# smartroboticslab/okvis2

Measured on AMD Instinct MI355X. Metric: front-end stereo-frames/s (detect+describe+match), 752x480 stereo, higher is better.
Workload: dtype u8/int32 (detect, describe, Hamming) + f64 (match gate); 1 GPU; EuRoC-shaped 752x480 stereo, euroc.yaml front-end params (radius 38, thr 150, <=700 kpts, match thr 60); lanes_per_gpu=1, score_kernels_serialised_across_lanes=False, stereo_frames_per_launch=3072, distinct_frames=256, content=corners, feed=device, cameras_per_multiframe=2, parallelism=frames sharded over 1 GPU(s), no collective

## Files before the change

### okvis2_amd/capi.py

```python
from __future__ import annotations

import ctypes as C
import os

import numpy as np

_HERE = os.path.dirname(os.path.abspath(__file__))
LIB_PATH = os.environ.get("OKVFE_LIB") or os.path.join(_HERE, "libokvfe.so")

OK = 0
ERR_INVALID_ARGUMENT, ERR_NO_DEVICE, ERR_OUT_OF_MEMORY, ERR_UNSUPPORTED, ERR_CAPACITY, ERR_DEVICE, \
    ERR_NOT_READY = 1, 2, 3, 4, 5, 6, 7
ABI_VERSION = 8
DIST_NONE, DIST_RADTAN, DIST_EQUIDISTANT, DIST_RADTAN8 = 0, 1, 2, 3
SCORE_HARRIS, SCORE_AGAST_9_16, SCORE_BRISK_SCALESPACE = 0, 1, 2
DESC_BYTES = 48

KEYPOINT_DTYPE = np.dtype([("x", "<f4"), ("y", "<f4"), ("size", "<f4"), ("angle", "<f4"),
                           ("response", "<f4"), ("octave", "<i4"), ("class_id", "<i4")])
STEREO_MATCH_DTYPE = np.dtype([("k1", "<i4"), ("dist", "<i4"), ("initialisable", "<i4"),
                               ("pad", "<i4"), ("hp_W", "<f8", (4,))])
CAND_DTYPE = np.dtype([("i", "<i4"), ("j", "<i4"), ("dist", "<i4")])
MOTION_MATCH_DTYPE = np.dtype([("k1", "<i4"), ("dist", "<i4"), ("initialisable", "<i4"),
                               ("accepted", "<i4"), ("cos_quality", "<f8"), ("hp_W", "<f8", (4,))])
# ... 48 lines not shown


class DeviceOutputs(C.Structure):
    _fields_ = [("max_keypoints", C.c_int32), ("counts", C.c_void_p), ("keypoints", C.c_void_p),
                ("descriptors", C.c_void_p), ("backproj", C.c_void_p),
                ("backproj_valid", C.c_void_p), ("scores", C.c_void_p),
                ("detect_counts", C.c_void_p), ("candidate_counts", C.c_void_p),
                ("score_pitch", C.c_int32), ("score_strips", C.c_int32)]


EXPORTS = [
    "okvfe_create", "okvfe_destroy", "okvfe_last_error", "okvfe_abi_version",
    "okvfe_set_camera_maps", "okvfe_set_camera", "okvfe_build_awareness_maps",
    "okvfe_detect_describe", "okvfe_detect", "okvfe_detect_ahead", "okvfe_detect_describe_batch_device",
    "okvfe_get_device_outputs", "okvfe_score_column", "okvfe_set_heavy_kernel_chaining", "okvfe_set_keep_score_map", "okvfe_set_internal_lanes", "okvfe_lanes_join", "okvfe_set_fp64_reduction", "okvfe_scale_index", "okvfe_download_image_result", "okvfe_harris_score_device", "okvfe_harris_byte_mover_device",
    "okvfe_match_stereo_batch_device", "okvfe_match_stereo", "okvfe_hamming_candidates",
    "okvfe_hamming_argmin", "okvfe_popcnt_xor", "okvfe_gather_block_bytes",
    "okvfe_pack_gather_block_device", "okvfe_match_stereo_blocks_device",
    "okvfe_profile_enable", "okvfe_profile_read", "okvfe_match_motion_stereo_blocks_device",
    "okvfe_detect_batch_device", "okvfe_describe_batch_device", "okvfe_camera_overlap", "okvfe_compute",
    "okvfe_match_motion_stereo", "okvfe_match_to_map",
    "okvfe_format_keypoint_lines", "okvfe_parse_keypoint_lines", "okvfe_fbrisk_mean",
    "okvfe_match_to_map_uninitialised", "okvfe_pack_gather_blocks_device",
    "okvfe_match_stereo_blocks_batch_device", "okvfe_check_capacity",
    "okvfe_detect_describe_batch_host", "okvfe_verify_place_match", "okvfe_fbrisk_transform",
    "okvfe_match_to_map_landmarks", "okvfe_bow_vector", "okvfe_bow_query_l1",
    "okvfe_get_pattern", "okvfe_set_pattern", "okvfe_pattern_kernel_class",
    "okvfe_match_to_map_blocks_device", "okvfe_match_to_map_uninitialised_blocks_device",
    "okvfe_verify_place_blocks_device",
    "okvfe_comm_unique_id", "okvfe_comm_create", "okvfe_comm_wrap", "okvfe_comm_destroy",
    "okvfe_comm_world", "okvfe_comm_rank", "okvfe_comm_last_error", "okvfe_gather_blocks",
    "okvfe_device_alloc", "okvfe_device_free", "okvfe_stream_create", "okvfe_stream_destroy",
    "okvfe_stream_synchronize", "okvfe_copy_to_device", "okvfe_copy_to_host", "okvfe_device_fill",
    "okvfe_set_camera_ext", "okvfe_build_awareness_maps_ext", "okvfe_camera_overlap_ext",
    "okvfe_match_motion_stereo_ext",
    "okvfe_keyframe_coverage_blocks_device", "okvfe_keyframe_coverage", "okvfe_keyframe_decision",
    "okvfe_landmark_table_check_device", "okvfe_match_to_map_table_blocks_device",
    "okvfe_match_to_map_table_uninitialised_blocks_device",
    "okvfe_ransac3d2d_consensus_blocks_device", "okvfe_remove_outliers_blocks_device",
    "okvfe_match_motion_stereo_blocks_batch_device",
    "okvfe_place_landmark_set", "okvfe_place_claims_blocks_device", "okvfe_place_consensus_blocks_device",
    "okvfe_place_hessian_blocks_device",
    "okvfe_vocabulary_check", "okvfe_bow_vectors_blocks_device", "okvfe_place_query_blocks_device",
    "okvfe_bow_database_add_blocks_device", "okvfe_bow_database_check_device",
    "okvfe_stereo_insert_blocks_device",
    "okvfe_ransac2d2d_consensus_blocks_device",
    "okvfe_overlap_pairs_blocks_device", "okvfe_overlap_fraction", "okvfe_motion_frame_order",
    "okvfe_tracking_quality",
    "okvfe_imu_propagation", "okvfe_imu_propagation_blocks_device",
]
TEST_HOOKS = [
    "okvfe_test_set_map_table_workspace_limit", "okvfe_test_ransac_chunk_records", "okvfe_test_ransac_ring_records",
    "okvfe_test_ransac2d2d_chunk_records", "okvfe_test_ransac2d2d_ring_records", "okvfe_test_ransac2d2d_id_slot",
    "okvfe_test_place_hessian_chunk_terms", "okvfe_test_context_sizes",
]

STAGES = ["harris", "nms", "sort", "select", "map", "describe", "compact", "match"]

_LIB = None


class LandmarkTable(C.Structure):
    _fields_ = [("n_landmarks", C.c_int32), ("n_observations", C.c_int32), ("n_poses", C.c_int32),
                ("hp_W", C.c_void_p), ("quality", C.c_void_p), ("obs_begin", C.c_void_p),
                ("obs_pose", C.c_void_p), ("obs_desc", C.c_void_p), ("obs_backproj", C.c_void_p),
                ("poses", C.c_void_p)]


class LandmarkPool(C.Structure):
    _fields_ = [("status", C.c_void_p), ("n_desc", C.c_void_p), ("obs_rows", C.c_void_p),
                ("projection", C.c_void_p), ("e_W", C.c_void_p), ("r_W", C.c_void_p)]


class LandmarkTableDevice(C.Structure):
    _fields_ = LandmarkTable._fields_


class LandmarkPoolDevice(C.Structure):
    _fields_ = LandmarkPool._fields_


class StereoInsertDevice(C.Structure):
    _fields_ = [("action", C.c_void_p), ("lm", C.c_void_p), ("landmark_out", C.c_void_p), ("counts", C.c_void_p)]


STEREO_MAX_PAIRS = 16
STEREO_REINIT, STEREO_CREATE, STEREO_OBS0, STEREO_OBS1 = 1, 2, 4, 8


class RansacResultDevice(C.Structure):
    _fields_ = [("n_correspondences", C.c_void_p), ("best_hypothesis", C.c_void_p), ("n_inliers", C.c_void_p),
                ("accepted", C.c_void_p), ("hyp_inliers", C.c_void_p), ("state", C.c_void_p),
                ("distance", C.c_void_p), ("landmark_out", C.c_void_p)]


class Ransac2d2dResultDevice(C.Structure):
    _fields_ = [(n, C.c_void_p) for n in (
        "n_correspondences", "rot_best", "rot_inliers", "rel_best", "rel_inliers", "branch", "removed",
        "total_inliers", "rotation_only", "success",
        "rot_hyp_inliers", "rel_hyp_inliers", "match1", "state", "distance", "landmark1_out")]


class PlaceSetDevice(C.Structure):
    _fields_ = [("n_landmarks", C.c_int32), ("hp", C.c_void_p)]


class PlaceClaimsDevice(C.Structure):
# ... 1043 lines not shown
            self._h, C.byref(database) if database is not None else None, _s(stream)))

    @staticmethod
    def _test_ransac_chunk_records() -> int:
        f = lib().okvfe_test_ransac_chunk_records
        f.restype = C.c_int32
        return int(f())

    @staticmethod
    def _test_place_hessian_chunk_terms() -> int:
        f = lib().okvfe_test_place_hessian_chunk_terms
        f.restype = C.c_int32
        return int(f())

    @staticmethod
    def _test_ransac2d2d_chunk_records() -> int:
        f = lib().okvfe_test_ransac2d2d_chunk_records
        f.restype = C.c_int32
        return int(f())

    @staticmethod
    def _test_ransac_ring_records() -> int:
        f = lib().okvfe_test_ransac_ring_records
        f.restype = C.c_int32
        return int(f())

    @staticmethod
    def _test_ransac2d2d_ring_records() -> int:
        f = lib().okvfe_test_ransac2d2d_ring_records
        f.restype = C.c_int32
        return int(f())

    @staticmethod
    def _test_ransac2d2d_id_slot(landmark_id) -> int:
        f = lib().okvfe_test_ransac2d2d_id_slot
        f.argtypes = [C.c_int32]
        f.restype = C.c_int32
        return int(f(int(landmark_id)))

    def _test_set_map_table_workspace_limit(self, nbytes):
        f = lib().okvfe_test_set_map_table_workspace_limit
        f.argtypes = [C.c_void_p, C.c_uint64]
        self._check(f(self._h, int(nbytes)))

    def _test_context_sizes(self, stream=None) -> dict:
        f = lib().okvfe_test_context_sizes
        f.argtypes = [C.c_void_p, C.c_void_p, C.POINTER(C.c_uint64)]
        out = (C.c_uint64 * 8)()
        self._check(f(self._h, _s(stream), out))
        keys = ("ring_slot_bytes", "ring_dev", "table_ws_bytes", "table_ws_dev", "perm_bytes", "perm_dev",
                "table_ws_entries", "perm_entries")
        return dict(zip(keys, (int(v) for v in out)))

    def verify_place_blocks_device(self, blocks_ptr, n_frames, map_dev, k_min_ptr, dist_min_ptr, stream=None):
        self._check(lib().okvfe_verify_place_blocks_device(
            self._h, _p(blocks_ptr), int(n_frames), C.byref(map_dev), _p(k_min_ptr), _p(dist_min_ptr),
            _s(stream)))

    def keyframe_coverage_blocks_device(self, blocks_ptr, n_frames, landmark_ids_ptr, coverage_ptr, id_set_ptr=None,
                                        n_id_set=0, kptrad=KPTRAD, stream=None):
        self._check(lib().okvfe_keyframe_coverage_blocks_device(
            self._h, _p(blocks_ptr), int(n_frames), _p(landmark_ids_ptr), _p(id_set_ptr), int(n_id_set),
            C.c_double(kptrad), _p(coverage_ptr), _s(stream)))

    def keyframe_coverage(self, keypoints, landmark_ids, id_set=None, kptrad=KPTRAD):
        kps = np.ascontiguousarray(keypoints, dtype=KEYPOINT_DTYPE)
        ids = np.ascontiguousarray(landmark_ids, dtype=np.uint64)
        if len(ids) != len(kps):
            raise ValueError("landmark_ids: one per keypoint")
        s = None if id_set is None else np.ascontiguousarray(id_set, dtype=np.uint64).reshape(-1)
        if s is not None and len(s) == 0:
            s = np.zeros(1, dtype=np.uint64)
            n_set = 0
        else:
            n_set = 0 if s is None else len(s)
        out = np.zeros(1, dtype=COVERAGE_DTYPE)
        self._check(lib().okvfe_keyframe_coverage(self._h, _p(kps) if len(kps) else None, len(kps),
                                                  _p(ids) if len(ids) else None, _p(s), n_set,
                                                  C.c_double(kptrad), _p(out)))
        return out[0]

    def overlap_pairs_blocks_device(self, blocks_ptr, block_stride_m, block_stride_c, n_multiframes, n_cams,
                                    landmark_ids_ptr, pair_a, pair_b, counts_ptr, coverage_ptr=None, kptrad=KPTRAD,
                                    stream=None):
        a = np.ascontiguousarray(pair_a, dtype=np.int32).reshape(-1)
        b = np.ascontiguousarray(pair_b, dtype=np.int32).reshape(-1)
        if len(a) != len(b):
            raise ValueError("pair_a / pair_b: one multiframe index each per pair")
        n = len(a)
        self._check(lib().okvfe_overlap_pairs_blocks_device(
            self._h, _p(blocks_ptr), int(block_stride_m), int(block_stride_c), int(n_multiframes), int(n_cams),
            _p(landmark_ids_ptr), _p(a) if n else None, _p(b) if n else None, n, C.c_double(kptrad), _p(counts_ptr),
            _p(coverage_ptr), _s(stream)))

    def gather_block_bytes(self) -> int:
        return int(lib().okvfe_gather_block_bytes(self._h))

    def pack_gather_block_device(self, index, block_ptr, stream=None):
        self._check(lib().okvfe_pack_gather_block_device(self._h, int(index), _p(block_ptr),
                                                         _s(stream)))

    def pack_gather_blocks_device(self, first, n, blocks_ptr, stream=None):
        self._check(lib().okvfe_pack_gather_blocks_device(self._h, int(first), int(n),
                                                          _p(blocks_ptr), _s(stream)))

    def match_stereo_blocks_batch_device(self, blocks0_ptr, blocks1_ptr, n_frames, T0, T1, f0, f1,
# ... 43 lines not shown
```

### okvis2_amd/csrc/capi_match.cpp

```cpp
#include "okvfe_ctx.h"

using namespace okvfe;

extern "C" {

okvfe_status okvfe_match_stereo_batch_device(okvfe_ctx* ctx, const okvfe_stereo_pair* pairs,
                                             int32_t n_pairs, okvfe_stereo_match* matches_dev,
                                             void* stream) {
  if (!ctx) return OKVFE_ERR_INVALID_ARGUMENT;
  if (!pairs || !matches_dev || n_pairs < 1)
    return fail(ctx, OKVFE_ERR_INVALID_ARGUMENT, "okvfe_match_stereo_batch_device: bad argument");
  HIP_TRY(ctx, hipSetDevice(ctx->cfg.device));
  std::vector<PairParams> pp(n_pairs);
  for (int i = 0; i < n_pairs; ++i) {
    if (pairs[i].image0 < 0 || pairs[i].image0 >= ctx->B || pairs[i].image1 < 0 || pairs[i].image1 >= ctx->B ||
        !(pairs[i].f0 > 0.0) || !(pairs[i].f1 > 0.0))
      return fail(ctx, OKVFE_ERR_INVALID_ARGUMENT, "pair %d: image index or focal length out of range", i);
    pp[i] = to_pair_params(pairs[i]);
  }
  std::vector<int> lane_first;
  bool piped = ctx->lanes_pipelined && ctx->lanes_open && ctx->n_layers == 1 && ctx->lane_chunk > 0 &&
               ctx->lanes_used > 1 && (int)ctx->lane_ctx.size() >= ctx->lanes_used && ctx->join_stream;
  if (piped) {
    lane_first.assign(ctx->lanes_used + 1, n_pairs);
// ... 427 lines not shown
                    fn, i1, user[i1], p);
      user[i1] = p;
    }
    rt8 = rt8 || dc.distortion == OKVFE_DIST_RADTAN8;
    okvfe_stereo_pair sp{};
    sp.T_WC0 = T_WC0[p]; sp.T_WC1 = T_WC1[p];
    sp.f0 = sp.f1 = 0.5 * (dc.fu + dc.fv);
    recs[p].pair = to_pair_params(sp);
    recs[p].cam = cam; recs[p].idx0 = i0; recs[p].idx1 = i1; recs[p].pad = 0;
    size_t j = 0;
    while (j < slots.size() && slots[j] != cam) ++j;
    if (j == slots.size()) slots.push_back(cam);
    slot_of[p] = (int)j;
  }
  if (claim && ctx->kp_cap > kMotionClaimMaxKeypoints)
    return fail(ctx, OKVFE_ERR_UNSUPPORTED, "%s: claims need max_keypoints <= %d (this context: %d)", fn,
                kMotionClaimMaxKeypoints, ctx->kp_cap);
  HIP_TRY(ctx, hipSetDevice(ctx->cfg.device));
  hipStream_t s = pick_stream(ctx, stream);
  const BlockLayout L = block_layout(ctx->kp_cap);
  okvfe_status st;
  RingSlot cls(ctx, &ctx->cls_ring, s), rec(ctx, &ctx->pair_ring, s);
  if (ctx->n_layers > 1) {
    std::vector<double> tables(slots.size() * kClassTableDoubles);
    for (size_t j = 0; j < slots.size(); ++j) {
      const DeviceCamera& dc = ctx->h_cams[slots[j]];
      const double f = 0.5 * (dc.fu + dc.fv);
      fill_class_table(tables.data() + j * kClassTableDoubles, f, f, true);
    }
    if ((st = cls.upload(tables.data(), tables.size() * sizeof(double))) != OKVFE_OK) return st;
    for (int p = 0; p < n_pairs; ++p) recs[p].pair.cls = cls.as<double>() + (size_t)slot_of[p] * kClassTableDoubles;
  }
  if ((st = rec.upload(recs.data(), recs.size() * sizeof(MotionPairRecord))) != OKVFE_OK) return st;
  launch_match_motion_pairs(rec.as<MotionPairRecord>(), n_pairs, ctx->d_cams, ctx->w, ctx->h, L,
                            static_cast<const uint8_t*>(blocks0_dev), static_cast<const uint8_t*>(blocks1_dev),
                            skip0_dev, matched1_dev, ctx->kp_cap, ctx->cfg.match_threshold, matches_dev, s, rt8);
  if (claim)
    launch_motion_claim(rec.as<MotionPairRecord>(), n_pairs, L,
                        static_cast<const uint8_t*>(blocks0_dev), ctx->kp_cap, matches_dev, claim->claimed,
                        claim->n_claimed, claim->matched1_out, s);
  HIP_TRY(ctx, hipGetLastError());
  ctx->last_stream = s;
  if ((st = rec.release()) != OKVFE_OK) return st;
  return cls.release();
}

okvfe_status okvfe_match_stereo_blocks_device(okvfe_ctx* ctx, const void* block0_dev, const void* block1_dev,
                                              const okvfe_pose* T_WC0, const okvfe_pose* T_WC1, double f0,
                                              double f1, okvfe_stereo_match* matches_dev, void* stream) {
  return okvfe_match_stereo_blocks_batch_device(ctx, block0_dev, block1_dev, 1, T_WC0, T_WC1, f0, f1, matches_dev,
                                                stream);
}

}
```

### okvis2_amd/csrc/k_match.hip

```cpp
#include "camera_dev.h"
#include <algorithm>
#include <cassert>

#include "okvfe_internal.h"
#include "bow_dev.h"

namespace okvfe {
namespace {

__device__ int g_fp64_tree = 1;
__device__ __forceinline__ double sum3(double p0, double p1, double p2) {
  const bool tree = g_fp64_tree != 0;
  const double u = tree ? p1 : p0, v = tree ? p2 : p1, w = tree ? p0 : p2;
  const double s = u + v;
  return tree ? w + s : s + w;
}
__device__ __forceinline__ double dot3(const double a[3], const double b[3]) {
  const double p0 = a[0] * b[0];
  const double p1 = a[1] * b[1];
  const double p2 = a[2] * b[2];
  return sum3(p0, p1, p2);
}
__device__ __forceinline__ void normalize3(const double v[3], double out[3]) {
  const double n = sqrt(dot3(v, v));
  out[0] = v[0] / n;
  out[1] = v[1] / n;
  out[2] = v[2] / n;
}
__device__ __forceinline__ void rot(const double C[9], const double v[3], double out[3]) {
  out[0] = dot3(C, v);
  out[1] = dot3(C + 3, v);
  out[2] = dot3(C + 6, v);
}
__device__ __forceinline__ void rot_t(const double C[9], const double v[3], double out[3]) {
#pragma unroll
  for (int i = 0; i < 3; ++i) {
    const double p0 = C[i] * v[0];
    const double p1 = C[3 + i] * v[1];
    const double p2 = C[6 + i] * v[2];
    out[i] = sum3(p0, p1, p2);
  }
}
__device__ __forceinline__ void inv_transform_h(const double C[9], const double r[3],
                                                const double hp[4], double out[4]) {
  double cr[3], h[3];
  rot_t(C, r, cr);
  rot_t(C, hp, h);
  const double s = hp[3];
  out[0] = h[0] + (-cr[0]) * s;
  out[1] = h[1] + (-cr[1]) * s;
  out[2] = h[2] + (-cr[2]) * s;
  out[3] = s;
}

__device__ void midpoint_parallel(const double p1[3], const double e1[3], const double p2[3],
                                  const double e2[3], const double t12[3], double c26,
                                  double hp[4], bool* is_valid) {
  *is_valid = true;
// ... 124 lines not shown
__device__ __forceinline__ uint32_t hamming_chain(const Desc12& a, const uint32_t* __restrict__ b) {
  uint32_t c = bcnt_first(a.w[0] ^ b[0]);
#pragma unroll
  for (int i = 1; i < 12; ++i) c = bcnt_acc(a.w[i] ^ b[i], c);
  return c;
}
template <int K, bool HAS_SKIP, bool FLOOR>
__device__ __forceinline__ void scan_top(const Desc12& d0, const ScanChunk& C,
                                         const uint8_t* __restrict__ desc1,
                                         const uint8_t* __restrict__ skip1, int k1_lo, int k1_hi,
                                         bool resident, uint32_t floor_key, uint32_t threshold,
                                         uint32_t (&c)[K]) {
  const uint32_t lim = (min(threshold, kMaxDist + 1u) << 22) + 1u;
  const uint32_t base = FLOOR ? floor_key + 1u : 0u;
  const uint32_t lim_u = lim - base;
#pragma unroll
  for (int t = 0; t < K; ++t) c[t] = lim_u;
  for (int c0 = k1_lo; c0 < k1_hi; c0 += kStereoChunk) {
    const int cnt = min(kStereoChunk, k1_hi - c0);
    if (!resident) load_scan_chunk(C, desc1, HAS_SKIP ? skip1 : nullptr, c0, cnt);
    auto insert = [&](uint32_t dist, int jj) {
      const uint32_t low = HAS_SKIP ? C.low[jj] : (uint32_t)(c0 + jj + 1);
      uint32_t key = (dist << 22) | low;
      if (FLOOR) key -= base;
#pragma unroll
      for (int t = K - 1; t > 0; --t) c[t] = med3_u32(c[t - 1], c[t], key);
      c[0] = min(c[0], key);
    };
    int j = 0;
    for (; j + 4 <= cnt; j += 4) {
#pragma unroll
      for (int u = 0; u < 4; ++u)
        insert(hamming_chain(d0, reinterpret_cast<const uint32_t*>(C.desc + 3 * (j + u))), j + u);
    }
    for (; j < cnt; ++j)
      insert(hamming_chain(d0, reinterpret_cast<const uint32_t*>(C.desc + 3 * j)), j);
  }
#pragma unroll
  for (int t = 0; t < K; ++t) c[t] = c[t] < lim_u ? c[t] + base : kNoKey;
}
static_assert(kNarrowScans == 1, "scan_top2 is the floor-free form: only a lane's first scan may use it");
template <bool HAS_SKIP>
__device__ __forceinline__ void scan_top2(const Desc12& d0, const ScanChunk& C,
                                          const uint8_t* __restrict__ desc1,
                                          const uint8_t* __restrict__ skip1, int k1_lo, int k1_hi,
                                          bool resident, uint32_t threshold,
                                          uint32_t* c1_out, uint32_t* c2_out) {
  uint32_t c[2];
  scan_top<2, HAS_SKIP, false>(d0, C, desc1, skip1, k1_lo, k1_hi, resident, 0u, threshold, c);
  *c1_out = c[0];
  *c2_out = c[1];
}

__device__ void match_stereo_rows(const PairParams& P, const BlockView& I0, const BlockView& I1,
                                  int threshold, okvfe_stereo_match* __restrict__ out) {
  constexpr int kMore = OKVFE_MATCH_MORE;
  __shared__ uint4 seg_desc[kStereoSegs][kStereoChunk * 3];
  __shared__ uint32_t best_key[64];
  __shared__ double e0_lds[3][64];
  __shared__ uint32_t job_key[64 * kStereoSegs];
  __shared__ uint8_t job_who[64 * kStereoSegs];
  __shared__ uint8_t job_res[kStereoSegs][64];
  __shared__ double hp_lds[kStereoSegs][4][64];
  __shared__ int seg_out[kStereoSegs][3][64];
  __shared__ int job_n[2];
  const int seg = __builtin_amdgcn_readfirstlane(threadIdx.y);
  const int lane = threadIdx.x;
  const int tid = seg * 64 + lane;
  const int per_seg = (I1.n + kStereoSegs - 1) / kStereoSegs;
  const int k1_lo = min(seg * per_seg, I1.n), k1_hi = min(k1_lo + per_seg, I1.n);
  if ((int)blockIdx.x * 64 >= I0.n) return;
  const int k0 = blockIdx.x * 64 + lane;
  const bool active = k0 < I0.n;
  Desc12 d0 = {};
  if (active) d0 = load_desc(I0.desc + (size_t)k0 * OKVFE_DESC_BYTES);
  const bool v0 = active && I0.bpv[k0] != 0;
  if (seg == 0) {
    double e[3] = {0, 0, 0};
    if (v0) {
      double v[3];
      rot(P.C0, I0.bp + 3 * (size_t)k0, v);
      normalize3(v, e);
    }
    e0_lds[0][lane] = e[0]; e0_lds[1][lane] = e[1]; e0_lds[2][lane] = e[2];
    best_key[lane] = kNoKey;
    if (lane < 2) job_n[lane] = 0;
  }
  const ScanChunk chunk{seg_desc[seg], nullptr};
  const bool resident = k1_hi - k1_lo <= kStereoChunk;
  if (resident) load_scan_chunk(chunk, I1.desc, nullptr, k1_lo, k1_hi - k1_lo);
  enum { kDone = 0, kHave = 1, kNeedScan = 2 };
  int state = v0 ? kNeedScan : kDone;
  uint32_t cs[kMore];
#pragma unroll
  for (int u = 0; u < kMore; ++u) cs[u] = kNoKey;
  int t = 0, n_c = 2, n_scans = 0;
  uint32_t floor_key = 0;
  int best = threshold, k1_match = 0, initialisable = 0;
  int par = 0;
  __syncthreads();
  while (true) {
    if (!__any(state == kHave) && __any(state == kNeedScan)) {
      if (n_scans < kNarrowScans) {
        scan_top2<false>(d0, chunk, I1.desc, nullptr, k1_lo, k1_hi, resident, (uint32_t)threshold, &cs[0], &cs[1]);
#pragma unroll
        for (int u = 2; u < kMore; ++u) cs[u] = kNoKey;
        n_c = 2;
      } else {
        scan_top<kMore, false, true>(d0, chunk, I1.desc, nullptr, k1_lo, k1_hi, resident, floor_key, (uint32_t)threshold, cs);
        n_c = kMore;
      }
      ++n_scans;
      t = 0;
      if (state == kNeedScan) state = kHave;
    }
    uint32_t cand = cs[0];
#pragma unroll
    for (int u = 1; u < kMore; ++u) cand = t == u ? cs[u] : cand;
    if (state == kHave && cand == kNoKey) state = kDone;
    if (state == kHave && cand > *reinterpret_cast<volatile uint32_t*>(&best_key[lane])) state = kDone;
    const bool pending = state == kHave;
    {
      const unsigned long long m = __ballot(pending);
      if (m != 0ull) {
        int base = 0;
        if (lane == 0) base = atomicAdd(&job_n[par], __popcll(m));
        base = __builtin_amdgcn_readfirstlane(base);
        if (pending) {
          const int at = base + __popcll(m & ((1ull << lane) - 1ull));
          job_key[at] = cand;
          job_who[at] = (uint8_t)(seg << 6 | lane);
        }
      }
    }
    if (!__syncthreads_or(state != kDone)) break;
    const int J = job_n[par];
    if (J > 0) {
      if (tid == 0) job_n[par ^ 1] = 0;
      if (seg * 64 < J) {
        const bool on = tid < J;
        const uint32_t key = on ? job_key[tid] : 1u;
        const int who = on ? job_who[tid] : 0;
        const int jl = who & 63, js = who >> 6;
        const int k1 = (int)((key - 1u) & 0x3FFFFFu);
        bool is_valid = false, is_parallel = false;
        double hp_W[4] = {0, 0, 0, 0};
        if (on && I1.bpv[k1]) {
          const int jk0 = blockIdx.x * 64 + jl;
          const double e0_W[3] = {e0_lds[0][jl], e0_lds[1][jl], e0_lds[2][jl]};
          double v[3], e1_W[3], hp_C0[4], hp_C1[4];
          rot(P.C1, I1.bp + 3 * (size_t)k1, v);
          normalize3(v, e1_W);
          double c26, c6;
          gate_cos(P, I0.kps, jk0, I1.kps, k1, &c26, &c6);
          triangulate_fast(P.r0, e0_W, P.r1, e1_W, c26, c6, hp_W, &is_valid, &is_parallel);
          inv_transform_h(P.C0, P.r0, hp_W, hp_C0);
          inv_transform_h(P.C1, P.r1, hp_W, hp_C1);
// ... 24 lines not shown
          initialisable = (r & 2) ? 0 : 1;
          state = kDone;
        } else {
          ++t;
          if (t >= n_c) state = kNeedScan;
        }
      }
      par ^= 1;
    }
  }
  seg_out[seg][0][lane] = best;
  seg_out[seg][1][lane] = k1_match;
  seg_out[seg][2][lane] = initialisable;
  __syncthreads();
  if (seg > 0 || !active) return;
  int win = 0;
#pragma unroll
  for (int s2 = 1; s2 < kStereoSegs; ++s2) {
    const int b2 = seg_out[s2][0][lane];
    if (b2 < best) {
      best = b2; k1_match = seg_out[s2][1][lane]; initialisable = seg_out[s2][2][lane];
      win = s2;
    }
  }
  okvfe_stereo_match m;
  const bool hit = best < threshold;
  m.k1 = hit ? k1_match : -1;
  m.dist = hit ? best : threshold;
  m.initialisable = hit ? initialisable : 0;
  m.pad = 0;
  m.hp_W[0] = hit ? hp_lds[win][0][lane] : 0.0;
  m.hp_W[1] = hit ? hp_lds[win][1][lane] : 0.0;
  m.hp_W[2] = hit ? hp_lds[win][2][lane] : 0.0;
  m.hp_W[3] = hit ? hp_lds[win][3][lane] : 0.0;
  out[k0] = m;
}


__global__ __launch_bounds__(64 * kStereoSegs) __attribute__((amdgpu_waves_per_eu(OKVFE_MATCH_WAVES, 8))) void match_stereo_kernel(
    const PairParams* __restrict__ pairs, const okvfe_keypoint* __restrict__ kps,
    const uint8_t* __restrict__ desc, const double* __restrict__ bp,
    const uint8_t* __restrict__ bpv, const int32_t* __restrict__ counts, int kp_cap,
    int threshold, okvfe_stereo_match* __restrict__ out) {
  const PairParams& P = pairs[blockIdx.y];
  BlockView I0, I1;
  const size_t o0 = (size_t)P.image0 * kp_cap, o1 = (size_t)P.image1 * kp_cap;
  I0.desc = desc + o0 * OKVFE_DESC_BYTES; I0.bp = bp + o0 * 3; I0.bpv = bpv + o0;
  I0.n = counts[P.image0]; I0.kps = kps + o0;
  I1.desc = desc + o1 * OKVFE_DESC_BYTES; I1.bp = bp + o1 * 3; I1.bpv = bpv + o1;
  I1.n = counts[P.image1]; I1.kps = kps + o1;
  match_stereo_rows(P, I0, I1, threshold, out + (size_t)blockIdx.y * kp_cap);
}

__global__ __launch_bounds__(64 * kStereoSegs) __attribute__((amdgpu_waves_per_eu(4, 8))) void match_stereo_arrays_kernel(
    const PairParams* __restrict__ pair, const uint8_t* __restrict__ desc0,
    const double* __restrict__ bp0, const uint8_t* __restrict__ bpv0, const int32_t* n0p, int n0,
    const uint8_t* __restrict__ desc1, const double* __restrict__ bp1,
    const uint8_t* __restrict__ bpv1, const int32_t* n1p, int n1, int threshold,
    okvfe_stereo_match* __restrict__ out, const okvfe_keypoint* __restrict__ kp0,
    const okvfe_keypoint* __restrict__ kp1) {
  BlockView I0, I1;
  I0.desc = desc0; I0.bp = bp0; I0.bpv = bpv0; I0.n = n0p ? *n0p : n0; I0.kps = kp0;
  I1.desc = desc1; I1.bp = bp1; I1.bpv = bpv1; I1.n = n1p ? *n1p : n1; I1.kps = kp1;
  match_stereo_rows(*pair, I0, I1, threshold, out);
}

__global__ __launch_bounds__(64) void hamming_argmin_kernel(const uint8_t* __restrict__ A, int nA,
                                                            const uint8_t* __restrict__ B, int nB,
                                                            uint32_t thr,
                                                            int32_t* __restrict__ best_j,
                                                            uint32_t* __restrict__ best_d) {
  const int i = blockIdx.x * 64 + threadIdx.x;
  if (i >= nA) return;
  const Desc12 a = load_desc(A + (size_t)i * OKVFE_DESC_BYTES);
  uint32_t dmin = thr;
  int jmin = -1;
  for (int j = 0; j < nB; ++j) {
    const uint32_t d =
        (uint32_t)hamming(a, reinterpret_cast<const uint32_t*>(B + (size_t)j * OKVFE_DESC_BYTES));
    if (d < dmin) {
      dmin = d;
      jmin = j;
    }
  }
  best_j[i] = jmin;
  best_d[i] = dmin;
}

__global__ __launch_bounds__(64) void hamming_count_kernel(const uint8_t* __restrict__ A, int nA,
                                                           const uint8_t* __restrict__ B, int nB,
                                                           int thr, int32_t* __restrict__ rows) {
  const int i = blockIdx.x * 64 + threadIdx.x;
  if (i >= nA) return;
  const Desc12 a = load_desc(A + (size_t)i * OKVFE_DESC_BYTES);
  int c = 0;
  for (int j = 0; j < nB; ++j)
    c += hamming(a, reinterpret_cast<const uint32_t*>(B + (size_t)j * OKVFE_DESC_BYTES)) < thr;
  rows[i] = c;
}

__global__ __launch_bounds__(64) void hamming_emit_kernel(const uint8_t* __restrict__ A, int nA,
                                                          const uint8_t* __restrict__ B, int nB,
                                                          int thr,
                                                          const int32_t* __restrict__ offsets,
                                                          okvfe_candidate* __restrict__ out,
                                                          int cap) {
// ... 1069 lines not shown
                         const int32_t* counts, int kp_cap, int threshold,
                         okvfe_stereo_match* out, hipStream_t stream) {
  if (n_pairs <= 0) return;
  check_scan_range(kp_cap);
  hipLaunchKernelGGL(match_stereo_kernel, dim3((kp_cap + 63) / 64, n_pairs), dim3(64, kStereoSegs), 0, stream,
                     pairs, kps, desc, bp, bpv, counts, kp_cap, threshold, out);
}

void launch_match_stereo_arrays(const PairParams* pair, const uint8_t* desc0, const double* bp0,
                                const uint8_t* bpv0, const int32_t* n0p, int n0,
                                const uint8_t* desc1, const double* bp1, const uint8_t* bpv1,
                                const int32_t* n1p, int n1, int max_rows, int threshold,
                                okvfe_stereo_match* out, hipStream_t stream, const okvfe_keypoint* kp0,
                                const okvfe_keypoint* kp1) {
  if (max_rows <= 0) return;
  check_scan_range(n1);
  hipLaunchKernelGGL(match_stereo_arrays_kernel, dim3((max_rows + 63) / 64), dim3(64, kStereoSegs), 0, stream,
                     pair, desc0, bp0, bpv0, n0p, n0, desc1, bp1, bpv1, n1p, n1, threshold, out, kp0, kp1);
}

void launch_verify_place(const uint8_t* pool, const int32_t* desc_begin, int n_landmarks,
                         const uint8_t* frame_desc, int K, uint32_t threshold, int32_t* k_min,
                         uint32_t* dist_min, hipStream_t stream) {
  if (n_landmarks <= 0) return;
  const int blocks = std::min((n_landmarks + 3) / 4, 2048);
  hipLaunchKernelGGL(verify_place_kernel, dim3(blocks), dim3(256), 0, stream, pool, desc_begin, n_landmarks,
                     frame_desc, K, threshold, k_min, dist_min, MapBatch{});
}
void launch_verify_place_blocks(const uint8_t* pool, const int32_t* desc_begin, int n_landmarks, const BlockLayout& L,
                                const uint8_t* blocks, int n_frames, int kp_cap, uint32_t threshold,
                                int32_t* k_min, uint32_t* dist_min, hipStream_t stream) {
  if (n_landmarks <= 0 || n_frames <= 0) return;
  const int blocks_x = std::min((n_landmarks + 3) / 4, 2048);
  const MapBatch mb = map_batch(blocks, L, kp_cap, 0);
  hipLaunchKernelGGL(verify_place_kernel, dim3(blocks_x, n_frames), dim3(256), 0, stream, pool, desc_begin,
                     n_landmarks, nullptr, 0, threshold, k_min, dist_min, mb);
}
void launch_bow_query_l1(const int32_t* db_begin, const int32_t* db_ids, const double* db_values, int n_entries,
                         const int32_t* q_ids, const double* q_values, int n_q, double* scores,
                         hipStream_t stream) {
  if (n_entries <= 0) return;
  hipLaunchKernelGGL(bow_query_l1_kernel, dim3((n_entries + 255) / 256), dim3(256), 0, stream, db_begin, db_ids,
                     db_values, n_entries, q_ids, q_values, n_q, scores);
}

void launch_voc_transform(const uint8_t* desc, int n, const uint8_t* node_desc, int n_nodes,
                          const int32_t* child_begin, const int32_t* child_index, const int32_t* word,
                          int32_t* word_out, int32_t* node_out, hipStream_t stream) {
  if (n <= 0) return;
  hipLaunchKernelGGL(voc_transform_kernel, dim3((n + 255) / 256), dim3(256), 0, stream, desc, n, node_desc,
                     n_nodes, child_begin, child_index, word, word_out, node_out);
}

void launch_hamming_argmin(const uint8_t* A, int nA, const uint8_t* B, int nB, uint32_t thr,
                           int32_t* best_j, uint32_t* best_d, hipStream_t stream) {
  if (nA <= 0) return;
  hipLaunchKernelGGL(hamming_argmin_kernel, dim3((nA + 63) / 64), dim3(64), 0, stream, A, nA, B,
                     nB, thr, best_j, best_d);
}

void launch_hamming_count(const uint8_t* A, int nA, const uint8_t* B, int nB, int thr,
                          int32_t* row_counts, hipStream_t stream) {
  if (nA <= 0) return;
  hipLaunchKernelGGL(hamming_count_kernel, dim3((nA + 63) / 64), dim3(64), 0, stream, A, nA, B,
                     nB, thr, row_counts);
}

void launch_hamming_emit(const uint8_t* A, int nA, const uint8_t* B, int nB, int thr,
                         const int32_t* row_offsets, okvfe_candidate* out, int cap,
                         hipStream_t stream) {
  if (nA <= 0) return;
  hipLaunchKernelGGL(hamming_emit_kernel, dim3((nA + 63) / 64), dim3(64), 0, stream, A, nA, B, nB,
                     thr, row_offsets, out, cap);
}

bool set_fp64_tree_match(int tree) {
  const int v = tree != 0;
  return hipMemcpyToSymbol(HIP_SYMBOL(g_fp64_tree), &v, sizeof(v)) == hipSuccess;
}

}
```

### okvis2_amd/csrc/okvfe_internal.h

```cpp
#pragma once
#include <cstddef>
#include <atomic>
#include <cstdlib>

#include <hip/hip_runtime.h>
#include <stdint.h>

#include <string>
#include <vector>

#include "../../include/okvfe.h"
#include "imu_dev.h"

namespace okvfe {

#ifdef OKVFE_LAB
inline const char* lab_env(const char* name) { return std::getenv(name); }
#else
inline const char* lab_env(const char*) { return nullptr; }
#endif

constexpr int kMaxAttrDevices = 64;
struct PerDeviceOnce {
  std::atomic<int> state[kMaxAttrDevices];
// ... 465 lines not shown
                         int min_inliers, const okvfe_place_claims_device& out, hipStream_t stream);
void launch_place_consensus(const double* hp, int n_landmarks, const BlockLayout& L, const uint8_t* blocks, int n_multiframes,
                            int n_cams, int kp_cap, const RansacCamParams* cams, const int32_t* match_landmark,
                            const uint8_t* gate, const double* hypotheses, const uint8_t* hyp_valid, int n_hyp,
                            double threshold, int min_inliers, const okvfe_ransac_result_device& out, uint8_t* verdict,
                            hipStream_t stream);
struct HessianCamParams {
  double pose[7];
  int32_t cam;
  int32_t pad;
};
static_assert(sizeof(HessianCamParams) == 64, "64 bytes per camera");
struct PlaceHessianArgs {
  const double* hp;
  int n_landmarks;
  const uint8_t* blocks;
  int o_count, o_kps;
  size_t block_bytes;
  int kp_cap, n_cams, w, h;
  const HessianCamParams* cams;
  const DeviceCamera* dcams;
  const double* poses;
  const int32_t* match_landmark;
  const uint8_t* state;
  const uint8_t* verdict;
  double* H;
  int32_t *n_terms, *n_singular;
  double *residual, *jacobian;
};
void launch_place_hessian(const PlaceHessianArgs& args, int n_multiframes, bool rt8, hipStream_t stream);
int place_hessian_chunk_terms();
bool set_fp64_tree_place_hessian(int tree);
constexpr int kImuRigHeaderDoubles = 8;
struct ImuArgs {
  const double* samples;
  const int32_t* sample_begin;
  const double* states;
  const double* rig;
  int n_multiframes, n_cams;
  ImuResultPtrs out;
};
void launch_imu_propagation(const ImuArgs& args, hipStream_t stream);
bool set_fp64_tree_imu(int tree);
void launch_halfsample(const uint8_t* src, int w, int h, int n_images, uint8_t* dst, hipStream_t stream);
void launch_twothird(const uint8_t* src, int w, int h, int n_images, uint8_t* dst, hipStream_t stream);
void launch_scale_filter(Candidate* cand, int cand_cap, int32_t* cand_count, int n_images,
                         const int32_t* below, ScoreLayout lb, int wb, int hb, int rn_b, int rd_b,
                         const int32_t* above, ScoreLayout la, int wa, int ha, int rn_a, int rd_a,
                         hipStream_t stream);
void launch_merge_layers(const okvfe_keypoint* const* kps, const int32_t* const* counts,
                         const int32_t* const* cand_counts, const int* cand_cap, const float* scale, int n_layers,
                         int layer_cap, int n_images, okvfe_keypoint* out, int out_cap,
                         int32_t* out_count, hipStream_t stream);
void launch_hamming_argmin(const uint8_t* A, int nA, const uint8_t* B, int nB, uint32_t thr,
                           int32_t* best_j, uint32_t* best_d, hipStream_t stream);
void launch_hamming_count(const uint8_t* A, int nA, const uint8_t* B, int nB, int thr,
                          int32_t* row_counts, hipStream_t stream);
void launch_hamming_emit(const uint8_t* A, int nA, const uint8_t* B, int nB, int thr,
                         const int32_t* row_offsets, okvfe_candidate* out, int cap,
                         hipStream_t stream);
constexpr int kCoverageMaxRadius = 127;
constexpr size_t kCoverageLdsBudget = 64 * 1024 - 256;
struct CoverageArgs {
  const uint8_t* base;
  size_t frame_stride;
  int o_count, o_kps;
  int kp_limit;
  const uint64_t* ids;
  size_t id_stride;
  const uint64_t* id_set;
  int n_id_set, has_set;
  int log2_slots;
  int rows, cols, r;
  uint8_t hw[kCoverageMaxRadius + 1];
};
void circle_half_widths(int r, uint8_t* hw);
struct CoverageGeometry {
  int rows, cols, r;
  int log2_slots;
  size_t lds;
  uint8_t hw[kCoverageMaxRadius + 1];
};
void launch_keyframe_coverage(const CoverageArgs& args, int n_frames, size_t lds_bytes, okvfe_coverage* out,
                              hipStream_t stream);
constexpr int kOverlapMaxCams = 32;
constexpr size_t kOverlapCountsLds = 2 * kOverlapMaxCams * sizeof(int32_t);
struct OverlapArgs {
  const uint8_t* blocks;
  size_t block_bytes;
  int o_count, o_kps, kp_cap;
  const uint64_t* ids;
  const int32_t* pairs;
  int stride_m, stride_c, n_cams;
  int tiles;
  int log2_slots;
  int rows, cols, r;
  okvfe_overlap_counts* counts;
  okvfe_coverage* coverage;
  uint8_t hw[kCoverageMaxRadius + 1];
};
void launch_overlap_pairs(const OverlapArgs& args, int n_pairs, size_t lds_bytes, hipStream_t stream);

constexpr int kBowMaxFeatures = 8192;
constexpr size_t kBowLdsBudget = 61 * 1024;
constexpr int kBowDenseWords = 4096;
constexpr int kBowQueryLdsWords = 4096;
// ... 46 lines not shown
```

Before: 828,000 stereo-frames/s.

## Compute stereo first-scan Hamming top-2 with int8 MFMA instead of popcount scan

Replaces the first narrow popcount scan in stereo matching with a matrix-core pass. Descriptor bits are expanded into signed int8 bit-planes and multiplied with mfma_i32_32x32x32_i8, so the dot product encodes the Hamming distance. Per-segment top-2 keys are reduced into shared memory with atomicMin. It applies when the threshold is at most 160 (the config uses 60) and adds a test probe kernel that compares the result against the scalar scan. The cost is 12 MFMAs per 32x64 tile, bit-plane expansion work, extra LDS and shared-memory atomics, while the scalar path still handles later scans.

```diff
diff --git a/okvis2_amd/capi.py b/okvis2_amd/capi.py
--- a/okvis2_amd/capi.py
+++ b/okvis2_amd/capi.py
@@ -124,7 +124,7 @@
 TEST_HOOKS = [
     "okvfe_test_set_map_table_workspace_limit", "okvfe_test_ransac_chunk_records", "okvfe_test_ransac_ring_records",
     "okvfe_test_ransac2d2d_chunk_records", "okvfe_test_ransac2d2d_ring_records", "okvfe_test_ransac2d2d_id_slot",
-    "okvfe_test_place_hessian_chunk_terms", "okvfe_test_context_sizes",
+    "okvfe_test_place_hessian_chunk_terms", "okvfe_test_context_sizes", "okvfe_test_stereo_first_scan_keys",
 ]
 
 STAGES = ["harris", "nms", "sort", "select", "map", "describe", "compact", "match"]
@@ -1274,6 +1274,11 @@
                 "table_ws_entries", "perm_entries")
         return dict(zip(keys, (int(v) for v in out)))
 
+    def _test_stereo_first_scan_keys(self, desc0_ptr, n0, desc1_ptr, n1, threshold, keys_ptr, stream=None):
+        f = lib().okvfe_test_stereo_first_scan_keys
+        f.argtypes = [C.c_void_p, C.c_void_p, C.c_int32, C.c_void_p, C.c_int32, C.c_int32, C.c_void_p, C.c_void_p]
+        self._check(f(self._h, _p(desc0_ptr), int(n0), _p(desc1_ptr), int(n1), int(threshold), _p(keys_ptr), _s(stream)))
+
     def verify_place_blocks_device(self, blocks_ptr, n_frames, map_dev, k_min_ptr, dist_min_ptr, stream=None):
         self._check(lib().okvfe_verify_place_blocks_device(
             self._h, _p(blocks_ptr), int(n_frames), C.byref(map_dev), _p(k_min_ptr), _p(dist_min_ptr),
diff --git a/okvis2_amd/csrc/capi_match.cpp b/okvis2_amd/csrc/capi_match.cpp
--- a/okvis2_amd/csrc/capi_match.cpp
+++ b/okvis2_amd/csrc/capi_match.cpp
@@ -503,4 +503,18 @@
                                                 stream);
 }
 
-}
+okvfe_status okvfe_test_stereo_first_scan_keys(okvfe_ctx* ctx, const void* desc0_dev, int32_t n0, const void* desc1_dev,
+                                               int32_t n1, int32_t threshold, void* keys_dev, void* stream) {
+  if (!ctx) return OKVFE_ERR_INVALID_ARGUMENT;
+  if (!desc0_dev || !desc1_dev || !keys_dev || n0 < 0 || n1 < 0 || n1 > ((1 << 22) - 1) || threshold < 0 || threshold > 385)
+    return fail(ctx, OKVFE_ERR_INVALID_ARGUMENT, "okvfe_test_stereo_first_scan_keys: bad argument");
+  HIP_TRY(ctx, hipSetDevice(ctx->cfg.device));
+  hipStream_t s = pick_stream(ctx, stream);
+  launch_first_scan_probe(static_cast<const uint8_t*>(desc0_dev), n0, static_cast<const uint8_t*>(desc1_dev), n1,
+                          threshold, static_cast<uint32_t*>(keys_dev), s);
+  HIP_TRY(ctx, hipGetLastError());
+  ctx->last_stream = s;
+  return OKVFE_OK;
+}
+
+}
diff --git a/okvis2_amd/csrc/hamming_mfma_dev.h b/okvis2_amd/csrc/hamming_mfma_dev.h
--- /dev/null
+++ b/okvis2_amd/csrc/hamming_mfma_dev.h
@@ -0,0 +1,30 @@
+#pragma once
+#include <hip/hip_runtime.h>
+#include <stdint.h>
+
+namespace okvfe {
+
+typedef int ham_v4i __attribute__((ext_vector_type(4)));
+typedef int ham_v16i __attribute__((ext_vector_type(16)));
+
+constexpr int kHamUnit = 64 * 64;
+constexpr int kHamBits = 384;
+
+__device__ __forceinline__ int ham_half_shift(int lane) { return (lane & 32) ? 0 : 4; }
+
+__device__ __forceinline__ ham_v4i ham_planes(uint32_t u) {
+  ham_v4i r;
+  r[0] = (int)(((u << 3) & 0x80808080u) | 0x40404040u);
+  r[1] = (int)(((u << 2) & 0x80808080u) | 0x40404040u);
+  r[2] = (int)(((u << 1) & 0x80808080u) | 0x40404040u);
+  r[3] = (int)((u & 0x80808080u) | 0x40404040u);
+  return r;
+}
+
+__device__ __forceinline__ int ham_acc_row(int v, int lane) { return 8 * (v >> 2) + 4 * (lane >> 5) + (v & 3); }
+
+__device__ __forceinline__ int ham_dist(int dot) { return (kHamBits - (dot >> 12)) >> 1; }
+
+__device__ __forceinline__ int ham_dot_bound(int thr_eff) { return kHamUnit * (kHamBits - 2 * (thr_eff - 1)); }
+
+}
diff --git a/okvis2_amd/csrc/k_match.hip b/okvis2_amd/csrc/k_match.hip
--- a/okvis2_amd/csrc/k_match.hip
+++ b/okvis2_amd/csrc/k_match.hip
@@ -4,6 +4,7 @@
 
 #include "okvfe_internal.h"
 #include "bow_dev.h"
+#include "hamming_mfma_dev.h"
 
 namespace okvfe {
 namespace {
@@ -234,10 +235,77 @@
   *c2_out = c[1];
 }
 
+#ifndef OKVFE_MATCH_MFMA_MAX_THR
+#define OKVFE_MATCH_MFMA_MAX_THR 160
+#endif
+constexpr uint32_t kMfmaMaxThr = OKVFE_MATCH_MFMA_MAX_THR;
+__device__ __forceinline__ void mfma_first_scan(const BlockView& I0, const BlockView& I1, int per_seg, int thr_eff,
+                                                uint32_t (*top2)[64][2]) {
+  const int wave = __builtin_amdgcn_readfirstlane(threadIdx.y);
+  const int lane = threadIdx.x;
+  const int sh = ham_half_shift(lane);
+  const int q = (wave & 1) * 32 + (lane & 31);
+  const int k0 = blockIdx.x * 64 + q;
+  ham_v4i qf[12];
+  {
+    const uint4* src = reinterpret_cast<const uint4*>(I0.desc + (size_t)min(k0, I0.n - 1) * OKVFE_DESC_BYTES);
+#pragma unroll
+    for (int p = 0; p < 3; ++p) {
+      const uint4 w = src[p];
+      qf[4 * p + 0] = ham_planes(w.x << sh);
+      qf[4 * p + 1] = ham_planes(w.y << sh);
+      qf[4 * p + 2] = ham_planes(w.z << sh);
+      qf[4 * p + 3] = ham_planes(w.w << sh);
+    }
+  }
+  const int bound = ham_dot_bound(thr_eff);
+  const int ntiles = (I1.n + 31) >> 5;
+  auto tile_src = [&](int tile) {
+    return reinterpret_cast<const uint4*>(I1.desc + (size_t)min(tile * 32 + (lane & 31), I1.n - 1) * OKVFE_DESC_BYTES);
+  };
+  const int seg1 = per_seg, seg2 = 2 * per_seg, seg3 = 3 * per_seg;
+  uint4 w[3];
+  if ((wave >> 1) < ntiles) {
+    const uint4* src = tile_src(wave >> 1);
+    w[0] = src[0]; w[1] = src[1]; w[2] = src[2];
+  }
+  for (int tile = wave >> 1; tile < ntiles; tile += 2) {
+    const uint4* next = tile_src(min(tile + 2, ntiles - 1));
+    const uint4 nw[3] = {next[0], next[1], next[2]};
+    ham_v16i acc = {};
+#pragma unroll
+    for (int p = 0; p < 3; ++p) {
+      acc = __builtin_amdgcn_mfma_i32_32x32x32_i8(ham_planes(w[p].x << sh), qf[4 * p + 0], acc, 0, 0, 0);
+      acc = __builtin_amdgcn_mfma_i32_32x32x32_i8(ham_planes(w[p].y << sh), qf[4 * p + 1], acc, 0, 0, 0);
+      acc = __builtin_amdgcn_mfma_i32_32x32x32_i8(ham_planes(w[p].z << sh), qf[4 * p + 2], acc, 0, 0, 0);
+      acc = __builtin_amdgcn_mfma_i32_32x32x32_i8(ham_planes(w[p].w << sh), qf[4 * p + 3], acc, 0, 0, 0);
+    }
+    w[0] = nw[0]; w[1] = nw[1]; w[2] = nw[2];
+    int top = acc[0];
+#pragma unroll
+    for (int v = 1; v < 16; ++v) top = max(top, acc[v]);
+    if (__ballot(top >= bound) == 0ull) continue;
+    if (top >= bound && k0 < I0.n) {
+#pragma unroll
+      for (int v = 0; v < 16; ++v) {
+        const int k1 = tile * 32 + ham_acc_row(v, lane);
+        if (acc[v] >= bound && k1 < I1.n) {
+          const uint32_t key = ((uint32_t)ham_dist(acc[v]) << 22) | (uint32_t)(k1 + 1);
+          const int s = (k1 >= seg1) + (k1 >= seg2) + (k1 >= seg3);
+          uint32_t* slot = top2[s][q];
+          const uint32_t old = atomicMin(&slot[0], key);
+          atomicMin(&slot[1], max(old, key));
+        }
+      }
+    }
+  }
+}
+
 __device__ void match_stereo_rows(const PairParams& P, const BlockView& I0, const BlockView& I1,
                                   int threshold, okvfe_stereo_match* __restrict__ out) {
   constexpr int kMore = OKVFE_MATCH_MORE;
   __shared__ uint4 seg_desc[kStereoSegs][kStereoChunk * 3];
+  __shared__ uint32_t top2[kStereoSegs][64][2];
   __shared__ uint32_t best_key[64];
   __shared__ double e0_lds[3][64];
   __shared__ uint32_t job_key[64 * kStereoSegs];
@@ -254,9 +322,11 @@
   if ((int)blockIdx.x * 64 >= I0.n) return;
   const int k0 = blockIdx.x * 64 + lane;
   const bool active = k0 < I0.n;
-  Desc12 d0 = {};
-  if (active) d0 = load_desc(I0.desc + (size_t)k0 * OKVFE_DESC_BYTES);
   const bool v0 = active && I0.bpv[k0] != 0;
+  const uint32_t thr_eff = min((uint32_t)threshold, kMaxDist + 1u);
+  const bool first_by_mfma = thr_eff <= kMfmaMaxThr;
+  if (first_by_mfma)
+    for (int i = tid; i < kStereoSegs * 64 * 2; i += 64 * kStereoSegs) (&top2[0][0][0])[i] = kNoKey;
   if (seg == 0) {
     double e[3] = {0, 0, 0};
     if (v0) {
@@ -281,10 +351,21 @@
   int best = threshold, k1_match = 0, initialisable = 0;
   int par = 0;
   __syncthreads();
+  if (first_by_mfma) {
+    mfma_first_scan(I0, I1, per_seg, (int)thr_eff, top2);
+    __syncthreads();
+  }
+  Desc12 d0 = {};
+  if (active) d0 = load_desc(I0.desc + (size_t)k0 * OKVFE_DESC_BYTES);
   while (true) {
     if (!__any(state == kHave) && __any(state == kNeedScan)) {
       if (n_scans < kNarrowScans) {
-        scan_top2<false>(d0, chunk, I1.desc, nullptr, k1_lo, k1_hi, resident, (uint32_t)threshold, &cs[0], &cs[1]);
+        if (first_by_mfma) {
+          cs[0] = top2[seg][lane][0];
+          cs[1] = top2[seg][lane][1];
+        } else {
+          scan_top2<false>(d0, chunk, I1.desc, nullptr, k1_lo, k1_hi, resident, (uint32_t)threshold, &cs[0], &cs[1]);
+        }
 #pragma unroll
         for (int u = 2; u < kMore; ++u) cs[u] = kNoKey;
         n_c = 2;
@@ -415,6 +496,40 @@
   match_stereo_rows(P, I0, I1, threshold, out + (size_t)blockIdx.y * kp_cap);
 }
 
+__global__ __launch_bounds__(64 * kStereoSegs) void first_scan_probe_kernel(
+    const uint8_t* __restrict__ desc0, int n0, const uint8_t* __restrict__ desc1, int n1, int threshold,
+    uint32_t* __restrict__ keys) {
+  __shared__ uint4 seg_desc[kStereoSegs][kStereoChunk * 3];
+  __shared__ uint32_t top2[kStereoSegs][64][2];
+  BlockView I0, I1;
+  I0.desc = desc0; I0.bp = nullptr; I0.bpv = nullptr; I0.n = n0;
+  I1.desc = desc1; I1.bp = nullptr; I1.bpv = nullptr; I1.n = n1;
+  const int seg = __builtin_amdgcn_readfirstlane(threadIdx.y);
+  const int lane = threadIdx.x;
+  const int tid = seg * 64 + lane;
+  const int per_seg = (n1 + kStereoSegs - 1) / kStereoSegs;
+  const int k1_lo = min(seg * per_seg, n1), k1_hi = min(k1_lo + per_seg, n1);
+  if ((int)blockIdx.x * 64 >= n0) return;
+  const int k0 = blockIdx.x * 64 + lane;
+  const bool active = k0 < n0;
+  Desc12 d0 = {};
+  if (active) d0 = load_desc(desc0 + (size_t)k0 * OKVFE_DESC_BYTES);
+  const ScanChunk chunk{seg_desc[seg], nullptr};
+  const bool resident = k1_hi - k1_lo <= kStereoChunk;
+  if (resident) load_scan_chunk(chunk, desc1, nullptr, k1_lo, k1_hi - k1_lo);
+  uint32_t a, b;
+  scan_top2<false>(d0, chunk, desc1, nullptr, k1_lo, k1_hi, resident, (uint32_t)threshold, &a, &b);
+  for (int i = tid; i < kStereoSegs * 64 * 2; i += 64 * kStereoSegs) (&top2[0][0][0])[i] = kNoKey;
+  __syncthreads();
+  mfma_first_scan(I0, I1, per_seg, (int)min((uint32_t)threshold, kMaxDist + 1u), top2);
+  __syncthreads();
+  uint32_t* out = keys + (size_t)blockIdx.x * (2 * kStereoSegs * 64 * 2);
+  out[tid * 2 + 0] = active ? a : kNoKey;
+  out[tid * 2 + 1] = active ? b : kNoKey;
+  out[(kStereoSegs * 64 + tid) * 2 + 0] = top2[seg][lane][0];
+  out[(kStereoSegs * 64 + tid) * 2 + 1] = top2[seg][lane][1];
+}
+
 __global__ __launch_bounds__(64 * kStereoSegs) __attribute__((amdgpu_waves_per_eu(4, 8))) void match_stereo_arrays_kernel(
     const PairParams* __restrict__ pair, const uint8_t* __restrict__ desc0,
     const double* __restrict__ bp0, const uint8_t* __restrict__ bpv0, const int32_t* n0p, int n0,
@@ -1590,6 +1705,13 @@
                      n_nodes, child_begin, child_index, word, word_out, node_out);
 }
 
+void launch_first_scan_probe(const uint8_t* desc0, int n0, const uint8_t* desc1, int n1, int threshold,
+                             uint32_t* keys, hipStream_t stream) {
+  if (n0 <= 0) return;
+  hipLaunchKernelGGL(first_scan_probe_kernel, dim3((n0 + 63) / 64), dim3(64, kStereoSegs), 0, stream, desc0, n0,
+                     desc1, n1, threshold, keys);
+}
+
 void launch_hamming_argmin(const uint8_t* A, int nA, const uint8_t* B, int nB, uint32_t thr,
                            int32_t* best_j, uint32_t* best_d, hipStream_t stream) {
   if (nA <= 0) return;
diff --git a/okvis2_amd/csrc/okvfe_internal.h b/okvis2_amd/csrc/okvfe_internal.h
--- a/okvis2_amd/csrc/okvfe_internal.h
+++ b/okvis2_amd/csrc/okvfe_internal.h
@@ -541,6 +541,8 @@
                          const int32_t* const* cand_counts, const int* cand_cap, const float* scale, int n_layers,
                          int layer_cap, int n_images, okvfe_keypoint* out, int out_cap,
                          int32_t* out_count, hipStream_t stream);
+void launch_first_scan_probe(const uint8_t* desc0, int n0, const uint8_t* desc1, int n1, int threshold,
+                             uint32_t* keys, hipStream_t stream);
 void launch_hamming_argmin(const uint8_t* A, int nA, const uint8_t* B, int nB, uint32_t thr,
                            int32_t* best_j, uint32_t* best_d, hipStream_t stream);
 void launch_hamming_count(const uint8_t* A, int nA, const uint8_t* B, int nB, int thr,
```

Measured after the change: 833,600 stereo-frames/s (median of 6 runs). No clear change (+0.7%).
